# compix/Monte-Carlo-Raytracer

Measured on AMD Instinct MI355X. Metric: Mpaths/sec + achieved HBM GB/s, San-Miguel 1920x1080 at 1/2/4/8 MI355X, higher is better.
Workload: dtype f32; 1 GPU; san_miguel_proxy 1920x1080, unidirectional PT, maxDepth 2, random sampler, 1 spp per step, box-filter accumulate; width=1920, height=1080, triangles=9984786, max_depth=2, global_batch=1, bvh=RadeonRays-identical SAH, device build, parallelism=tile-split 8-row bands x 1 + 1 RCCL band gather, frames_per_launch=32, max_frames_per_call=32

## Files before the change

### monte-carlo-raytracer_amd/csrc/mcrt_kernels.hip

```cpp
#include <algorithm>

#include <rocprim/device/device_scan.hpp>

#include "mcrt_device.h"
#include "mcrt_internal.h"
#include "mcrt_traverse.h"
#include "mcrt_shading.h"

#ifndef SHADE0_BLOCK
#define SHADE0_BLOCK 512
#endif
#define SHADEN_BLOCK 256
#define MCRT_EXT_GROUPS 24

template <bool ANY, int LAY>
__global__ __launch_bounds__(64) void k_trace_rays(TraceCtx c, const mcrt_ray* __restrict__ rays, int n,
                                                   const int* __restrict__ countDev,
                                                   mcrt_intersection* __restrict__ hits, int* __restrict__ occl) {
    __shared__ __attribute__((aligned(16))) uint32_t lds[STACK_LDS * 64];
    if (countDev) n = min(n, *countDev);
    const int lane = threadIdx.x;
    const int i = blockIdx.x * 64 + lane;
    if (i >= n) return;
    const mcrt_ray rr = rays[i];
// ... 288 lines not shown

__global__ __launch_bounds__(64) void k_walk_resume(TraceCtx c, const float4* __restrict__ qO,
                                                    const float4* __restrict__ qD, float4* __restrict__ hitOut) {
    __shared__ __attribute__((aligned(16))) uint32_t lds[STACK_LDS * 64];
    const int n = *c.suspendCount;
    if ((int)blockIdx.x * 64 >= n) return;
    const int lane = threadIdx.x;
    const int j = blockIdx.x * 64 + lane;
    if (j >= n) return;
    const float4* sv = c.suspend + (size_t)j * MCRT_SUSPEND_F4;
    const float4 s0 = sv[0], s1 = sv[1];
    const int i = __float_as_int(s0.x);
    uint32_t* stk = lds + lane;
    uint32_t col = 0;
    for (int k = 0; k < STACK_LDS / 4; ++k) {
        const float4 e = sv[2 + k];
        if (k == 0) col = __float_as_uint(e.x);
        stk[(4 * k) * 64] = k == 0 ? QREF_DONE : __float_as_uint(e.x);
        stk[(4 * k + 1) * 64] = __float_as_uint(e.y);
        stk[(4 * k + 2) * 64] = __float_as_uint(e.z);
        stk[(4 * k + 3) * 64] = __float_as_uint(e.w);
    }
    QWalk w{__float_as_uint(s0.y), s0.z, s0.w, s1.x, __float_as_int(s1.y), __float_as_int(s1.z), __float_as_int(s1.w)};
    const float4 o = qO[i], d = qD[i];
    TraceRay r;
    r.o = ld3(o);
    r.d = ld3(d);
    r.tmax = RT_MAX_TRACE_F;
    r.mask = -1;
    uint32_t* spill = raySpill(c, (int)(col >> 6), (int)(col & 63));
    qwalk<false, -2>(c, r, safeInvDir(r.d), stk, spill, w);
    hitOut[i] = qwalkClosest(c, r, stk, spill, w);
}

template <int LAY0, int LAY1>
__global__ __launch_bounds__(64) void k_extend_pair(TraceCtx cc, TraceCtx c, const int* __restrict__ count0,
                                                    const float4* __restrict__ qO0, const float4* __restrict__ qD0,
                                                    float4* __restrict__ hit0, const int* __restrict__ count1,
                                                    const float4* __restrict__ qO1, const float4* __restrict__ qD1,
                                                    float4* __restrict__ hit1, const uint32_t* __restrict__ perm1) {
    __shared__ __attribute__((aligned(16))) uint32_t lds[STACK_LDS * 64];
    const int n0 = *count0;
    const int b0 = (n0 + 63) >> 6;
    const int lane = threadIdx.x;
    TraceRay r;
    r.tmax = RT_MAX_TRACE_F;
    r.mask = -1;
    float t;
    if ((int)blockIdx.x < b0) {
        const int blk = xcdRemap(blockIdx.x, b0);
        const int i = blk * 64 + lane;
        if (LAY0 == LAY_PLAIN && cc.packet) {
            const bool valid = i < n0;
            r.o = valid ? ld3(qO0[i]) : splat3(0.0f);
            r.d = valid ? ld3(qD0[i]) : f3{0.0f, 0.0f, 1.0f};
            const int tri = traversePacket<false>(cc.nodes, r, valid, t);
            if (valid) hit0[i] = closestRecord(cc.nodes, r, tri, t);
            return;
        }
        if (i >= n0) return;
        r.o = ld3(qO0[i]);
        r.d = ld3(qD0[i]);
        hit0[i] = traceClosest<LAY0>(cc, r, lds + lane, raySpill(cc, blk, lane), t);
    } else {
        const int n1 = *count1;
        const int b1 = (n1 + 63) >> 6;
        if ((int)blockIdx.x - b0 >= b1) return;
        const int j = xcdRemap((int)blockIdx.x - b0, b1) * 64 + lane;
        if (perm1 == nullptr) {
            if (j >= n1) return;
            r.o = ld3(qO1[j]);
            r.d = ld3(qD1[j]);
            closestOrSuspend<LAY1>(c, r, lds + lane, (int)blockIdx.x * 64 + lane, j, hit1);
            return;
        }
        if (j >= n1) return;
        const int i = (int)perm1[j];
        r.o = ld3(qO1[i]);
        r.d = ld3(qD1[i]);
        closestOrSuspend<LAY1>(c, r, lds + lane, (int)blockIdx.x * 64 + lane, i, hit1);
    }
}

struct ShadeOut {
    bool pushS, pushE;
    float4 sO, sD, sL;
    float4 eO, eD, eT;
};

template <bool LOD = false, bool EXT = true, bool RR = false>
MCRT_DEV f3 shadePath(const SceneArgs& s, const FrameArgs& f, int bounce, int pix, float4 hit, f3 dir, f3 throughput,
                      int prevFlags, ShadeOut& o, f3 ro = f3{0, 0, 0}, f3 dxDir = f3{0, 0, 0}, f3 dyDir = f3{0, 0, 0}) {
    f3 add = splat3(0.0f);
    const int shapeIdx = __float_as_int(hit.z), primIdx = __float_as_int(hit.w);
    if (shapeIdx < 0 || s.numLights <= 0) return add;
    const mcrt_shape shape = tableEntry(s.shapes, shapeIdx);
    f3 dpdu, dpdv;
    Frame si = computeSurfaceInteraction(s, shape, shapeIdx, primIdx, f2{hit.x, hit.y}, LOD ? &dpdu : nullptr,
                                         LOD ? &dpdv : nullptr);
    TexLod lod{{0.0f, 0.0f}, {0.0f, 0.0f}, false};
    if (LOD) lod = surfaceUVDifferentials(si, dpdu, dpdv, ro, dxDir, dyDir);
    const f3 wo = -dir;
    const bool isBackfacing = cl_dot(si.gn, wo) < 0.0f;
    const float traceErrorOffset = isBackfacing ? -RT_TRACE_OFFSET_F : RT_TRACE_OFFSET_F;
    const int materialId = shape.materialId;
    mcrt_material mat;
    if (materialId != -1) {
        mat = tableEntry(s.materials, materialId);
        if (mat.uber_normalMapId != -1) applyNormalMapping(s, mat.uber_normalMapId, si, lod);
    }
    if (bounce == 0) throughput = splat3(1.0f);
    if (shape.lightID != -1 && (bounce == 0 || (prevFlags & BSDF_SPECULAR) == BSDF_SPECULAR)) {
        const mcrt_light& L = s.lights[shape.lightID];
        f3 Le = splat3(0.0f);
        if ((L.type == MCRT_DISK_AREA_LIGHT || L.type == MCRT_TRIANGLE_MESH_AREA_LIGHT) && cl_dot(si.gn, wo) > 0.0f)
            Le = ld3(L.intensity);
        return throughput * Le;
    }
    int px = pix, frame = f.frame;
    if (f.batch > 1) {
        const int k = (int)((uint32_t)pix / (f.W * f.H));
        px = pix - k * (int)(f.W * f.H);
        frame += k;
    }
    Sampler sampler = makeSampler(f.sampler, (uint32_t)px, frame, bounce, f.W, f.H, s.sobol);
    const bool isUber = materialId != -1 && mat.type == 0;
    Uber um;
    if (isUber) um = uberProps(s, mat, si.uv, lod);
    {
        uint32_t lightIdx = (uint32_t)floorf(getSample1D(sampler) * s.numLights);
        lightIdx %= (uint32_t)s.numLights;
        const f2 u = getSample2D(sampler);
        const mcrt_light light = s.lights[lightIdx];
        const LightSample ls = sampleLightLi(s, light, si, traceErrorOffset, u);
        float lightPdf = ls.pdf * light.choicePdf;
        f3 L = splat3(0.0f);
        if (materialId != -1) {
            f3 bsdf = isUber ? evaluateUberBSDF(um, si, wo, ls.wi) : splat3(0.0f);
            bsdf *= absDot(ls.wi, si.sn);
            if (!isNearZero(lightPdf)) L = cl_div(ls.Li * bsdf, lightPdf);
        }
        const f3 term = throughput * L;
        if (term.x != 0.0f || term.y != 0.0f || term.z != 0.0f) {
            if (ls.shadowSet) {
                o.pushS = true;
                o.sO = make_float4(ls.shadowO.x, ls.shadowO.y, ls.shadowO.z, ls.shadowT);
                o.sD = make_float4(ls.wi.x, ls.wi.y, ls.wi.z, __int_as_float(pix));
                o.sL = make_float4(term.x, term.y, term.z, 0.0f);
            } else {
                add = term * 0.0f;
            }
        }
    }
    if (EXT && bounce + 1 < f.maxDepth) {
        const f2 bsdfSample = getSample2D(sampler);
        if (isUber) {
            f3 wi;
            float pdf;
            int sampledType;
            f3 bsdfBounce = sampleUberBSDF(um, si, bsdfSample, wo, &wi, &pdf, &sampledType);
            if (!(isNearZero(pdf) || isBlack(bsdfBounce))) {
                bsdfBounce = cl_div(bsdfBounce, pdf);
                const f3 tp = bsdfBounce * absDot(wi, si.sn);
                const f3 nt = throughput * tp;
                float off = traceErrorOffset;
                if ((sampledType & BSDF_TRANSMISSION) != 0 && cl_dot(si.gn, wi) * cl_sign(off) < 0.0f) off *= -1.0f;
                const f3 no = si.p + si.gn * off;
                bool alive = true;
                f3 tp1 = nt;
                if (RR && bounce + 1 >= f.rrStartDepth) {
                    const float qr = fmaxf(0.05f, 1.0f - fmaxf(nt.x, fmaxf(nt.y, nt.z)));
                    const float ur = (float)wangHash((uint32_t)px * 9781u + (uint32_t)frame * 6271u + (uint32_t)bounce) * 0x1p-32f;
                    alive = ur >= qr;
                    tp1 = cl_div(nt, (1.0f - qr));
                }
                if (alive) {
                    o.pushE = true;
                    o.eO = make_float4(no.x, no.y, no.z, __int_as_float(pix));
                    o.eD = make_float4(wi.x, wi.y, wi.z, __int_as_float(sampledType));
                    o.eT = make_float4(tp1.x, tp1.y, tp1.z, 0.0f);
                }
            }
        }
    }
    return add;
}

template <bool LOD, bool RR>
__global__ __launch_bounds__(SHADE0_BLOCK) void k_shade0(SceneArgs s, FrameArgs f, const mcrt_camera* __restrict__ camp,
                                                const float4* __restrict__ hits, float4* __restrict__ radiance,
                                                QueueArgs q) {
    const int lane = threadIdx.x & 63;
    const int tileAll = orderedTileAll(f, xcdRemap(blockIdx.x, gridDim.x) * (SHADE0_BLOCK / 64) + (int)(threadIdx.x >> 6));
    int k, tile, pi = lane;
    if (f.shadePack && f.batch > 1) {
        packedPath(f, tileAll, lane, k, tile, pi);
    } else {
        splitTileFrame(f, tileAll, k, tile);
    }
    int x = 0, y = 0;
    bool valid = k < f.batch && tile < f.numTiles && tilePixel(f, tile, pi, x, y);
    __shared__ int ldsWave[SHADE0_BLOCK / 64 + 1];
    __shared__ int ldsGroup[MCRT_EXT_GROUPS + 1];
    ShadeOut o;
    o.pushS = o.pushE = false;
    o.eD = make_float4(0.0f, 0.0f, 0.0f, 0.0f);
    if (valid) {
        const mcrt_camera& cam = camp[k];
        const int pix = k * (int)(f.W * f.H) + y * (int)f.W + x;
        const f3 dir = cameraDir(cam, x, y);
        f3 dx = splat3(0.0f), dy = splat3(0.0f);
        if (LOD) cameraDiffDirs(cam, x, y, dx, dy);
        const f3 add = shadePath<LOD, true, RR>(s, f, 0, pix, hits[hitSlot(f, tile, pi, k, x, y)], dir, splat3(1.0f), 0,
                                                o, ld3(cam.pos), dx, dy);
        radiance[pix] = make_float4(add.x, add.y, add.z, 0.0f);
    }
    const int ss = blockAppend<SHADE0_BLOCK / 64>(q.shadowCount, o.pushS, ldsWave);
    if (o.pushS) { q.sO[ss] = o.sO; q.sD[ss] = o.sD; q.sL[ss] = o.sL; }
    int oct = (o.eD.x < 0.0f ? 1 : 0) | (o.eD.y < 0.0f ? 2 : 0) | (o.eD.z < 0.0f ? 4 : 0);
    {
        const float ax = fabsf(o.eD.x), ay = fabsf(o.eD.y), az = fabsf(o.eD.z);
        oct = oct * 3 + (ax >= ay && ax >= az ? 0 : ay >= az ? 1 : 2);
    }
    const int es = blockAppendGroupedLds<MCRT_EXT_GROUPS>(q.extCountOut, o.pushE, oct, ldsGroup);
    if (o.pushE) { q.eOout[es] = o.eO; q.eDout[es] = o.eD; q.eTout[es] = o.eT; }
}

template <bool LAST, bool RR>
__global__ __launch_bounds__(SHADEN_BLOCK) void k_shadeN(SceneArgs s, FrameArgs f, int bounce, const int* __restrict__ countIn,
                                                const float4* __restrict__ qO, const float4* __restrict__ qD,
                                                const float4* __restrict__ qT, const float4* __restrict__ hits,
                                                float4* __restrict__ radiance, QueueArgs q) {
    const int n = *countIn;
    __shared__ int ldsWave[SHADEN_BLOCK / 64 + 1];
    __shared__ int ldsGroup[(SHADEN_BLOCK / 64) * 8 + 1];
    if ((int)blockIdx.x * SHADEN_BLOCK >= n) return;
    const int i = xcdRemap(blockIdx.x, (n + SHADEN_BLOCK - 1) / SHADEN_BLOCK) * SHADEN_BLOCK + threadIdx.x;
    ShadeOut o;
    o.pushS = o.pushE = false;
    o.eD = make_float4(0.0f, 0.0f, 0.0f, 0.0f);
    if (i < n) {
        const float4 O = qO[i], D = qD[i], Tp = qT[i];
        const int pix = __float_as_int(O.w);
        const f3 add = shadePath<false, !LAST, RR>(s, f, bounce, pix, hits[i], ld3(D), ld3(Tp), __float_as_int(D.w), o);
        if (add.x != 0.0f || add.y != 0.0f || add.z != 0.0f || add.x != add.x) {
            float4 r = radiance[pix];
            r.x += add.x; r.y += add.y; r.z += add.z;
            radiance[pix] = r;
        }
    }
    const int ss = blockAppend<SHADEN_BLOCK / 64>(q.shadowCount, o.pushS, ldsWave);
    if (o.pushS) { q.sO[ss] = o.sO; q.sD[ss] = o.sD; q.sL[ss] = o.sL; }
    if (LAST) return;
    const int oct = (o.eD.x < 0.0f ? 1 : 0) | (o.eD.y < 0.0f ? 2 : 0) | (o.eD.z < 0.0f ? 4 : 0);
    const int es = blockAppendGrouped<SHADEN_BLOCK / 64, 8>(q.extCountOut, o.pushE, oct, ldsGroup);
    if (o.pushE) { q.eOout[es] = o.eO; q.eDout[es] = o.eD; q.eTout[es] = o.eT; }
}

__global__ __launch_bounds__(256) void k_aov(SceneArgs s, FrameArgs f, const mcrt_camera* __restrict__ camp,
                                             const float4* __restrict__ hits, int which, float4* __restrict__ out) {
    const int lane = threadIdx.x & 63;
    const int tile = (blockIdx.x * blockDim.x + threadIdx.x) >> 6;
    int x, y;
    if (tile >= f.numTiles || !tilePixel(f, tile, lane, x, y)) return;
    const int pix = y * (int)f.W + x;
    const int stride = which == MCRT_AOV_TEXTURE_LOD ? 3 : 1;
    float4* o = out + (size_t)pix * stride;
    for (int k = 0; k < stride; ++k) o[k] = make_float4(0.0f, 0.0f, 0.0f, 0.0f);
    const float4 hit = hits[hitSlot(f, tile, lane, 0, x, y)];
    const int shapeIdx = __float_as_int(hit.z), primIdx = __float_as_int(hit.w);
    if (shapeIdx < 0) return;
    const mcrt_camera& cam = *camp;
    f3 dpdu, dpdv, dx, dy;
    const Frame si = computeSurfaceInteraction(s, shapeIdx, primIdx, f2{hit.x, hit.y}, &dpdu, &dpdv);
    cameraDiffDirs(cam, x, y, dx, dy);
    TexLod L = surfaceUVDifferentials(si, dpdu, dpdv, ld3(cam.pos), dx, dy);
    const int materialId = s.shapes[shapeIdx].materialId;
    if (which == MCRT_AOV_TEXTURE_LOD) {
        float lod = 0.0f;
        f4 c = f4{0.0f, 0.0f, 0.0f, 0.0f};
        if (materialId != -1 && s.materials[materialId].uber_diffuseTexId != -1) {
            const int t = s.materials[materialId].uber_diffuseTexId;
            const mcrt_texture_desc tex = s.textures[t];
            lod = mipLod(tex, L.duvdx, L.duvdy);
            c = readTexLodDesc(s, tex, si.uv, lod);
        }
        o[0] = make_float4(L.duvdx.x, L.duvdx.y, L.duvdy.x, L.duvdy.y);
        o[1] = make_float4(lod, __int_as_float(shapeIdx), si.uv.x, si.uv.y);
        o[2] = make_float4(c.x, c.y, c.z, c.w);
    } else {
        L.on = f.textureLod != 0;
        if (materialId != -1 && s.materials[materialId].type == 0) {
            const Uber u = uberProps(s, s.materials[materialId], si.uv, L);
            o[0] = make_float4(u.Kd.x, u.Kd.y, u.Kd.z, u.opacity.x);
        }
    }
}

template <bool MOTION>
__device__ __forceinline__ void guidesPixel(const SceneArgs& s, const FrameArgs& f, const mcrt_camera* __restrict__ camp,
                                            const float4* __restrict__ hits, float4* __restrict__ normalPlane,
                                            float4* __restrict__ albedoDepth, const PrevPose* __restrict__ prev,
                                            float4* __restrict__ motion, float4* __restrict__ prevNormal) {
    const int lane = threadIdx.x & 63;
    const int tile = (blockIdx.x * blockDim.x + threadIdx.x) >> 6;
    int x, y;
    if (tile >= f.numTiles || !tilePixel(f, tile, lane, x, y)) return;
    const int pix = y * (int)f.W + x;
    const float4 hit = hits[hitSlot(f, tile, lane, 0, x, y)];
    const int shapeIdx = __float_as_int(hit.z), primIdx = __float_as_int(hit.w);
    if (shapeIdx < 0) {
        normalPlane[pix] = make_float4(0.0f, 0.0f, 0.0f, 0.0f);
        albedoDepth[pix] = make_float4(0.0f, 0.0f, 0.0f, -1.0f);
        if (MOTION) {
            motion[pix] = make_float4(0.0f, 0.0f, 0.0f, 0.0f);
            prevNormal[pix] = make_float4(0.0f, 0.0f, 0.0f, 0.0f);
        }
        return;
    }
    const mcrt_camera& cam = *camp;
    f3 dpdu, dpdv, dx, dy;
    const Frame si = computeSurfaceInteraction(s, shapeIdx, primIdx, f2{hit.x, hit.y}, &dpdu, &dpdv);
    cameraDiffDirs(cam, x, y, dx, dy);
    TexLod L = surfaceUVDifferentials(si, dpdu, dpdv, ld3(cam.pos), dx, dy);
    L.on = f.textureLod != 0;
    f3 kd = f3{0.0f, 0.0f, 0.0f};
    const int materialId = s.shapes[shapeIdx].materialId;
    if (materialId != -1 && s.materials[materialId].type == 0) kd = uberProps(s, s.materials[materialId], si.uv, L).Kd;
    const f3 v = si.p - ld3(cam.pos);
    f3 n = si.sn;
    float off = cl_dot(n, v);
    const bool flipped = off > 0.0f;
    if (flipped) {
        n = f3{-n.x, -n.y, -n.z};
        off = -off;
    }
    normalPlane[pix] = make_float4(n.x, n.y, n.z, off);
    albedoDepth[pix] = make_float4(kd.x, kd.y, kd.z, cl_length(v));
    if (MOTION) {
// ... 691 lines not shown
```

### monte-carlo-raytracer_amd/csrc/mcrt_shading.h

```cpp
#pragma once
#include "mcrt_device.h"
#include "mcrt_internal.h"

MCRT_DEV bool tilePixel(const FrameArgs& f, int tile, int lane, int& x, int& y) {
    const int tb = tile / f.tilesX, tx = tile - tb * f.tilesX;
    const int bpb = f.bandRows >> 3;
    const int gb = (tb / bpb) * bpb * f.numBands + f.bandIndex * bpb + (tb % bpb);
    x = tx * 8 + (lane & 7);
    y = gb * 8 + (lane >> 3);
    return x < (int)f.W && y < (int)f.H;
}

MCRT_DEV int orderedTileAll(const FrameArgs& f, int tileAll) {
    if (!f.tileOrder) return tileAll;
    const int slot = tileAll / f.batch, part = tileAll - slot * f.batch;
    return slot < f.numTiles ? (int)f.tileOrder[slot] * f.batch + part : tileAll;
}

MCRT_DEV void splitTileFrame(const FrameArgs& f, int tileAll, int& k, int& tile) {
    if (f.tileMajor) {
        tile = tileAll / f.batch;
        k = tileAll - tile * f.batch;
    } else {
        k = tileAll / f.numTiles;
// ... 76 lines not shown

MCRT_DEV f4 readTexLodDesc(const SceneArgs& s, const mcrt_texture_desc& tex, f2 uv, float lod) {
    if (lod < 1e-8f || tex.numMipLevels < 2) return readTexDesc(s, tex, uv);
    if (lod >= (float)(tex.numMipLevels - 1)) {
        mcrt_texture_desc top = tex;
        uint16_t w = tex.width, h = tex.height;
        int off = 0;
        for (int i = 0; i < tex.numMipLevels - 1; ++i) {
            off += w * h * 4;
            w = (uint16_t)max(w / 2, 1);
            h = (uint16_t)max(h / 2, 1);
        }
        top.width = 1;
        top.height = 1;
        top.memOffset += off;
        return readTexDesc(s, top, uv);
    }
    const int lower = (int)floorf(lod);
    uint16_t w = tex.width, h = tex.height;
    int off = 0;
    for (int i = 0; i < lower; ++i) {
        off += w * h * 4;
        w = (uint16_t)max(w / 2, 1);
        h = (uint16_t)max(h / 2, 1);
    }
    mcrt_texture_desc lo = tex, hi = tex;
    lo.width = w;
    lo.height = h;
    lo.memOffset += off;
    const int offHi = off + w * h * 4;
    hi.width = (uint16_t)max(w / 2, 1);
    hi.height = (uint16_t)max(h / 2, 1);
    hi.memOffset += offHi;
    const f4 v0 = readTexDesc(s, lo, uv), v1 = readTexDesc(s, hi, uv);
    const float t = lod - (float)lower;
    return f4{fmaf(v1.x - v0.x, t, v0.x), fmaf(v1.y - v0.y, t, v0.y), fmaf(v1.z - v0.z, t, v0.z),
              fmaf(v1.w - v0.w, t, v0.w)};
}

MCRT_DEV f4 readTexL(const SceneArgs& s, int texId, f2 uv, const TexLod& L) {
    if (!L.on) return readTex(s, texId, uv);
    const mcrt_texture_desc tex = tableEntry(s.textures, texId);
    return readTexLodDesc(s, tex, uv, mipLod(tex, L.duvdx, L.duvdy));
}

MCRT_DEV bool solve2x2(float a00, float a01, float a10, float a11, f2 B, f2* x) {
    const float det = a00 * a11 - a10 * a01;
    if (fabsf(det) < 1e-8f) return false;
    *x = f2{cl_div(a11 * B.x - a01 * B.y, det), cl_div(a00 * B.y - a10 * B.x, det)};
    return true;
}

MCRT_DEV void cameraDiffDirs(const mcrt_camera& cam, int x, int y, f3& dx, f3& dy) {
    const f2 r = f2{cl_div(1.0f, (float)cam.width), cl_div(1.0f, (float)cam.height)};
    const f2 uv = f2{(float)x * r.x, (float)y * r.y};
    dx = lerpDirection(ld3(cam.r00), ld3(cam.r10), ld3(cam.r11), ld3(cam.r01), uv.x + r.x, uv.y);
    dy = lerpDirection(ld3(cam.r00), ld3(cam.r10), ld3(cam.r11), ld3(cam.r01), uv.x, uv.y + r.y);
}

MCRT_DEV Uber uberProps(const SceneArgs& s, const mcrt_material& material, f2 uv, const TexLod& L = TexLod{{0, 0}, {0, 0}, false},
                        bool* nonDelta = nullptr) {
    Uber u;
    const f4 Kd_opacity = material.uber_diffuseTexId != -1 ? readTexL(s, material.uber_diffuseTexId, uv, L) : f4{1.0f, 1.0f, 1.0f, 1.0f};
    u.Kd = Kd_opacity.xyz * ld3(material.uber_kd);
    const f3 glossy = material.uber_glossyTexId != -1 ? readTexL(s, material.uber_glossyTexId, uv, L).xyz : splat3(1.0f);
    u.Ks = glossy * ld3(material.uber_ks);
    u.Kr = (material.uber_specReflectionTexId != -1 ? readTexL(s, material.uber_specReflectionTexId, uv, L).xyz : splat3(1.0f)) *
           ld3(material.uber_kr);
    u.Kt.xyz = (material.uber_transmissionTexId != -1 ? readTexL(s, material.uber_transmissionTexId, uv, L).xyz : splat3(1.0f)) *
               ld3(material.uber_kt);
    u.Kt.w = material.uber_kt.w;
    const f3 opTex = material.uber_opacityTexId != -1 ? readTexL(s, material.uber_opacityTexId, uv, L).xyz : splat3(1.0f);
    u.opacity = opTex * ld3(material.uber_opacity) * Kd_opacity.w;
    if (nonDelta) {
        const f3 Kd = material.uber_diffuseTexId != -1 ? Kd_opacity.xyz : ld3(material.uber_kd);
        const f3 Ks = material.uber_glossyTexId != -1 ? glossy : ld3(material.uber_ks);
        const f3 op = material.uber_opacityTexId != -1 ? opTex : ld3(material.uber_opacity);
        const f3 kd = Kd * op, ks = Ks * op;
        *nonDelta = !isBlack(kd) || !isBlack(ks);
    }
    u.roughness = material.uber_roughnessTexId != -1 ? readTexL(s, material.uber_roughnessTexId, uv, L).xy
                                                      : f2{material.uber_roughness.x, material.uber_roughness.y};
    u.eta = material.uber_iorTexId != -1 ? readTexL(s, material.uber_iorTexId, uv, L).x : material.uber_eta;
    u.roughness = f2{roughnessToAlpha(u.roughness.x), roughnessToAlpha(u.roughness.y)};
    return u;
}

template <int NW>
MCRT_DEV int blockAppend(int* counter, bool pred, int* ldsWave ) {
    const unsigned long long m = __ballot(pred);
    const int lane = threadIdx.x & 63, wv = threadIdx.x >> 6;
    if (lane == 0) ldsWave[wv] = __popcll(m);
    __syncthreads();
    if (threadIdx.x == 0) {
        int sum = 0;
        for (int w = 0; w < NW; ++w) {
            const int c = ldsWave[w];
            ldsWave[w] = sum;
            sum += c;
        }
        ldsWave[NW] = sum ? atomicAdd(counter, sum) : 0;
    }
    __syncthreads();
    const unsigned lo = (unsigned)m, hi = (unsigned)(m >> 32);
    const int prefix = __builtin_amdgcn_mbcnt_hi(hi, __builtin_amdgcn_mbcnt_lo(lo, 0u));
    const int slot = ldsWave[NW] + ldsWave[wv] + prefix;
    __syncthreads();
    return slot;
}

template <int NW, int G>
MCRT_DEV int blockAppendGrouped(int* counter, bool pred, int group, int* lds) {
    const int lane = threadIdx.x & 63, wv = threadIdx.x >> 6;
    unsigned long long mine = 0;
#pragma unroll
    for (int g = 0; g < G; ++g) {
        const unsigned long long m = __ballot(pred && group == g);
        if (g == group) mine = m;
        if (lane == 0) lds[g * NW + wv] = __popcll(m);
    }
    __syncthreads();
    if (threadIdx.x == 0) {
        int sum = 0;
        for (int i = 0; i < G * NW; ++i) {
            const int c = lds[i];
            lds[i] = sum;
            sum += c;
        }
        lds[G * NW] = sum ? atomicAdd(counter, sum) : 0;
    }
    __syncthreads();
    const int prefix = __builtin_amdgcn_mbcnt_hi((unsigned)(mine >> 32), __builtin_amdgcn_mbcnt_lo((unsigned)mine, 0u));
    const int slot = lds[G * NW] + (pred ? lds[group * NW + wv] : 0) + prefix;
    __syncthreads();
    return slot;
}

template <int G>
MCRT_DEV int blockAppendGroupedLds(int* counter, bool pred, int group, int* lds) {
    for (int g = threadIdx.x; g < G; g += blockDim.x) lds[g] = 0;
    __syncthreads();
    const int local = pred ? atomicAdd(&lds[group], 1) : 0;
    __syncthreads();
    if (threadIdx.x == 0) {
        int sum = 0;
        for (int g = 0; g < G; ++g) {
            const int c = lds[g];
            lds[g] = sum;
            sum += c;
        }
        lds[G] = sum ? atomicAdd(counter, sum) : 0;
    }
    __syncthreads();
    const int slot = lds[G] + (pred ? lds[group] : 0) + local;
    __syncthreads();
    return slot;
}

MCRT_DEV int waveAppend(int* counter, bool pred) {
    const unsigned long long m = __ballot(pred);
    if (m == 0) return 0;
    const int lane = threadIdx.x & 63;
    const int leader = __ffsll((long long)m) - 1;
    int base = 0;
    if (lane == leader) base = atomicAdd(counter, __popcll(m));
    base = __shfl(base, leader);
// ... 187 lines not shown
```

### monte-carlo-raytracer_amd/mcrt/lib.py

```python
import ctypes
import weakref
import os

import numpy as np

from . import PKG_DIR
from . import types as T

_DEFAULT_LIB = os.path.join(os.path.dirname(PKG_DIR), "libmcrt.so")
LIB_PATH = os.environ.get("MCRT_LIB_PATH") or _DEFAULT_LIB
HEADER = os.path.join(os.path.dirname(os.path.dirname(PKG_DIR)), "include", "mcrt_capi.h")

_c = ctypes
_vp = _c.c_void_p
_lib = None

SIGNATURES = {
    "mcrt_version": (_c.c_char_p, []),
    "mcrt_last_error": (_c.c_char_p, [_vp]),
    "mcrt_ctx_create": (_c.c_int, [_c.c_int, _c.POINTER(_vp)]),
    "mcrt_ctx_destroy": (_c.c_int, [_vp]),
    "mcrt_ctx_synchronize": (_c.c_int, [_vp]),
    "mcrt_ctx_set_stream": (_c.c_int, [_vp, _vp]),
    "mcrt_ctx_set_profiling": (_c.c_int, [_vp, _c.c_int]),
# ... 276 lines not shown
        return rec

    def builder(self):
        b = _c.c_int32()
        _check(lib().mcrt_accel_builder(self.h, _c.byref(b)), self.ctx.h)
        return b.value

    def info(self):
        nn, nb, ms, nt = _c.c_uint64(), _c.c_uint64(), _c.c_double(), _c.c_uint32()
        _check(lib().mcrt_accel_info(self.h, _c.byref(nn), _c.byref(nb), _c.byref(ms), _c.byref(nt)), self.ctx.h)
        return {"nodes": nn.value, "bytes": nb.value, "build_ms": ms.value, "triangles": nt.value}

    def update_lights(self, lights):
        self._lights = np.ascontiguousarray(lights)
        _check(lib().mcrt_scene_update_lights(self.h, _p(self._lights), len(self._lights)), self.ctx.h)

    def update_materials(self, mats):
        self._mats = np.ascontiguousarray(mats)
        _check(lib().mcrt_scene_update_materials(self.h, _p(self._mats), len(self._mats)), self.ctx.h)

    def update_shapes(self, shapes):
        self._shapes = np.ascontiguousarray(shapes)
        _check(lib().mcrt_scene_update_shapes(self.h, _p(self._shapes), len(self._shapes)), self.ctx.h)

    def update_transforms(self, shapes, world_to_local=None):
        self._shapes = np.ascontiguousarray(shapes)
        w2l = None if world_to_local is None else np.ascontiguousarray(world_to_local, np.float32)
        _check(lib().mcrt_accel_update_transforms(self.h, _p(self._shapes), len(self._shapes), _p(w2l)), self.ctx.h)

    def motion_snapshot(self):
        _check(lib().mcrt_scene_motion_snapshot(self.h), self.ctx.h)

    def update_info(self):
        path, ms = _c.c_int32(), _c.c_double()
        _check(lib().mcrt_accel_update_info(self.h, _c.byref(path), _c.byref(ms)), self.ctx.h)
        return {"path": path.value, "ms": ms.value}

    def trace_closest(self, rays_dev_ptr, n, hits_dev_ptr):
        _check(lib().mcrt_trace_closest(self.h, rays_dev_ptr, n, hits_dev_ptr), self.ctx.h)

    def trace_any(self, rays_dev_ptr, n, out_dev_ptr):
        _check(lib().mcrt_trace_any(self.h, rays_dev_ptr, n, out_dev_ptr), self.ctx.h)

    def trace_count(self, any_hit, rays_dev_ptr, count_dev_ptr, maxrays, out_dev_ptr, wait_event=None,
                    want_event=False):
        ev = _vp()
        f = lib().mcrt_trace_any_count if any_hit else lib().mcrt_trace_closest_count
        _check(f(self.h, rays_dev_ptr, count_dev_ptr, maxrays, out_dev_ptr, wait_event,
                 _c.byref(ev) if want_event else None), self.ctx.h)
        return ev.value if want_event else None

    def close(self):
        if self.h:
            lib().mcrt_scene_destroy(self.h)
            self.h = None

    def __del__(self):
        try:
            self.close()
        except Exception:
            pass


class FrameBuffer:
    def __init__(self, ctx, width, height):
        self.ctx = ctx
        self.W, self.H = width, height
        h = _vp()
        _check(lib().mcrt_framebuffer_create(ctx.h, width, height, _c.byref(h)), ctx.h)
        self.h = h
        ctx._adopt(self)

    def set_frames_in_flight(self, n):
        _check(lib().mcrt_framebuffer_set_frames_in_flight(self.h, n), self.ctx.h)

    def render(self, dscene, cam, frame=0, max_depth=2, sampler=T.SAMPLER_RANDOM, rr=False, rr_start=3,
               band_rows=8, num_bands=1, band_index=0, integrator=T.INTEGRATOR_PT, texture_lod=False):
        p = T.FrameParams(frame, max_depth, sampler, 1 if rr else 0, rr_start, band_rows, num_bands, band_index,
                          integrator, 1 if texture_lod else 0)
        cam = np.ascontiguousarray(cam)
        _check(lib().mcrt_render_frame(dscene.h, self.h, _p(cam), _c.byref(p)), self.ctx.h)

    def render_frames(self, dscene, cams, frame=0, max_depth=2, sampler=T.SAMPLER_RANDOM, rr=False, rr_start=3,
                      band_rows=8, num_bands=1, band_index=0, integrator=T.INTEGRATOR_PT):
        p = T.FrameParams(frame, max_depth, sampler, 1 if rr else 0, rr_start, band_rows, num_bands, band_index,
                          integrator, 0)
        cams = _records(cams)
        _check(lib().mcrt_render_frames(dscene.h, self.h, _p(cams), len(cams), _c.byref(p)), self.ctx.h)

    def accumulate_frames(self, filters, frame):
        filters = _records(filters)
        _check(lib().mcrt_accumulate_frames(self.h, _p(filters), len(filters), frame), self.ctx.h)

    def render_aov(self, dscene, cam, aov=T.AOV_ALBEDO, texture_lod=False):
        p = T.FrameParams(0, 1, T.SAMPLER_RANDOM, 0, 3, 8, 1, 0, T.INTEGRATOR_PT, 1 if texture_lod else 0)
        cam = np.ascontiguousarray(cam)
        shape = (self.H, self.W, 3, 4) if aov == T.AOV_TEXTURE_LOD else (self.H, self.W, 4)
        out = np.zeros(shape, np.float32)
        _check(lib().mcrt_render_aov(dscene.h, self.h, _p(cam), _c.byref(p), aov, _p(out)), self.ctx.h)
        return out

    def accumulate(self, filt, frame):
        filt = np.ascontiguousarray(filt)
        _check(lib().mcrt_accumulate(self.h, _p(filt), frame), self.ctx.h)

    def postprocess(self, denoise=False, radius=1, sigma_spatial=1.0, sigma_range=0.1, tonemap=False,
                    min_luminance=2.0):
        p = T.PostprocessParams(1 if denoise else 0, radius, sigma_spatial, sigma_range, 1 if tonemap else 0,
                                min_luminance)
        _check(lib().mcrt_postprocess(self.h, _c.byref(p)), self.ctx.h)

    def render_guides(self, dscene, cam, texture_lod=False, band_rows=8, num_bands=1, band_index=0):
        p = T.FrameParams(0, 1, T.SAMPLER_RANDOM, 0, 3, band_rows, num_bands, band_index, T.INTEGRATOR_PT,
                          1 if texture_lod else 0)
        cam = np.ascontiguousarray(cam)
        _check(lib().mcrt_render_guides(dscene.h, self.h, _p(cam), _c.byref(p)), self.ctx.h)

    def render_guides_motion(self, dscene, cam, texture_lod=False, band_rows=8, num_bands=1, band_index=0):
        p = T.FrameParams(0, 1, T.SAMPLER_RANDOM, 0, 3, band_rows, num_bands, band_index, T.INTEGRATOR_PT,
                          1 if texture_lod else 0)
        cam = np.ascontiguousarray(cam)
        _check(lib().mcrt_render_guides_motion(dscene.h, self.h, _p(cam), _c.byref(p)), self.ctx.h)

    def set_motion(self, motion_ptr, prev_normal_ptr):
        _check(lib().mcrt_framebuffer_set_motion(self.h, motion_ptr, prev_normal_ptr), self.ctx.h)

    def read_motion(self, which):
        out = np.zeros((self.H, self.W, 4), np.float32)
        _check(lib().mcrt_framebuffer_read_motion(self.h, which, _p(out), out.nbytes, None), self.ctx.h)
        return out

    def set_guides(self, normal_plane_ptr, albedo_depth_ptr):
        _check(lib().mcrt_framebuffer_set_guides(self.h, normal_plane_ptr, albedo_depth_ptr), self.ctx.h)

    def enable_moments(self, on=True):
        _check(lib().mcrt_framebuffer_set_moments_enabled(self.h, 1 if on else 0), self.ctx.h)

    def set_moments(self, m1m2_ptr, frames):
        _check(lib().mcrt_framebuffer_set_moments(self.h, m1m2_ptr, int(frames)), self.ctx.h)

    GUIDE_SHAPES = {T.GUIDE_NORMAL_PLANE: (4,), T.GUIDE_ALBEDO_DEPTH: (4,), T.GUIDE_MOMENTS: (2,),
                    T.GUIDE_FILTERED_VARIANCE: ()}

    def read_guides(self, which):
        out = np.zeros((self.H, self.W) + self.GUIDE_SHAPES[which], np.float32)
        _check(lib().mcrt_framebuffer_read_guides(self.h, which, _p(out), out.nbytes, None), self.ctx.h)
        return out

    def denoise_guided(self, levels=5, sigma_normal=0.1, sigma_depth=0.02, sigma_luminance=4.0, use_variance=True,
                       demodulate_albedo=True, tonemap=False, min_luminance=2.0):
        p = T.GuidedDenoiseParams(levels, sigma_normal, sigma_depth, sigma_luminance, 1 if use_variance else 0,
                                  1 if demodulate_albedo else 0, 1 if tonemap else 0, min_luminance)
        _check(lib().mcrt_denoise_guided(self.h, _c.byref(p)), self.ctx.h)

    def temporal_accumulate(self, cam, alpha=0.2, alpha_moments=0.2, max_history=32, min_history=4,
                            normal_threshold=0.1, plane_threshold=0.01, demodulate_albedo=True):
        p = T.TemporalParams(alpha, alpha_moments, max_history, min_history, normal_threshold, plane_threshold,
                             1 if demodulate_albedo else 0)
        cam = np.ascontiguousarray(cam)
        _check(lib().mcrt_temporal_accumulate(self.h, _p(cam), _c.byref(p)), self.ctx.h)

    def temporal_accumulate_motion(self, cam, alpha=0.2, alpha_moments=0.2, max_history=32, min_history=4,
                                   normal_threshold=0.1, plane_threshold=0.01, demodulate_albedo=True):
        p = T.TemporalParams(alpha, alpha_moments, max_history, min_history, normal_threshold, plane_threshold,
                             1 if demodulate_albedo else 0)
        cam = np.ascontiguousarray(cam)
        _check(lib().mcrt_temporal_accumulate_motion(self.h, _p(cam), _c.byref(p)), self.ctx.h)

    def temporal_reset(self):
# ... 205 lines not shown
```

Before: 1932 Mpaths/s.

## Split shading into direct and extension phases with piecewise material loads

Splits the monolithic shadePath into shadeDirect and shadeExtend, so the shadow-ray queue append happens before the BSDF sampling for the extension ray. Material records are now read in 16-byte pieces on demand instead of copying the full 128-byte struct, and throughput is loaded lazily from the queue. Empty asm 'pin' barriers are added to control scheduling and register live ranges. The goal is lower register pressure and less memory traffic in the shade kernels. In exchange, the ShadeState struct must carry the surface frame and Uber properties across the block-wide append, which may raise live registers at that point. It also adds a texture_lod option to the Python render_frames call.

```diff
diff --git a/monte-carlo-raytracer_amd/csrc/mcrt_kernels.hip b/monte-carlo-raytracer_amd/csrc/mcrt_kernels.hip
--- a/monte-carlo-raytracer_amd/csrc/mcrt_kernels.hip
+++ b/monte-carlo-raytracer_amd/csrc/mcrt_kernels.hip
@@ -394,15 +394,32 @@
     }
 }
 
-struct ShadeOut {
-    bool pushS, pushE;
-    float4 sO, sD, sL;
-    float4 eO, eD, eT;
+struct ShadowRay {
+    bool push;
+    float4 o, d, l;
 };
-
-template <bool LOD = false, bool EXT = true, bool RR = false>
-MCRT_DEV f3 shadePath(const SceneArgs& s, const FrameArgs& f, int bounce, int pix, float4 hit, f3 dir, f3 throughput,
-                      int prevFlags, ShadeOut& o, f3 ro = f3{0, 0, 0}, f3 dxDir = f3{0, 0, 0}, f3 dyDir = f3{0, 0, 0}) {
+struct ExtRay {
+    bool push;
+    float4 o, d, t;
+};
+struct ShadeState {
+    bool ext;
+    Frame si;
+    Uber um;
+    f3 wo;
+    float traceErrorOffset;
+    f2 bsdfSample;
+    int px, frame;
+};
+
+MCRT_DEV f3 pathThroughput(int bounce, const float4* throughputAt) {
+    return bounce == 0 ? splat3(1.0f) : ld3(*throughputAt);
+}
+
+template <bool LOD = false, bool EXT = true, bool LIGHT_IN_PLACE = true>
+MCRT_DEV f3 shadeDirect(const SceneArgs& s, const FrameArgs& f, int bounce, int pix, float4 hit, f3 dir,
+                        const float4* throughputAt, int prevFlags, ShadowRay& sr, ShadeState& st, f3 ro = f3{0, 0, 0},
+                        f3 dxDir = f3{0, 0, 0}, f3 dyDir = f3{0, 0, 0}) {
     f3 add = splat3(0.0f);
     const int shapeIdx = __float_as_int(hit.z), primIdx = __float_as_int(hit.w);
     if (shapeIdx < 0 || s.numLights <= 0) return add;
@@ -410,24 +427,30 @@
     f3 dpdu, dpdv;
     Frame si = computeSurfaceInteraction(s, shape, shapeIdx, primIdx, f2{hit.x, hit.y}, LOD ? &dpdu : nullptr,
                                          LOD ? &dpdv : nullptr);
+    pin(si.p); pin(si.gn); pin(si.sn); pin(si.sdpdu); pin(si.sdpdv); pin(si.uv);
     TexLod lod{{0.0f, 0.0f}, {0.0f, 0.0f}, false};
-    if (LOD) lod = surfaceUVDifferentials(si, dpdu, dpdv, ro, dxDir, dyDir);
-    const f3 wo = -dir;
+    if (LOD) {
+        lod = surfaceUVDifferentials(si, dpdu, dpdv, ro, dxDir, dyDir);
+        pin(lod.duvdx); pin(lod.duvdy);
+    }
+    f3 wo = -dir;
+    pin(wo);
     const bool isBackfacing = cl_dot(si.gn, wo) < 0.0f;
     const float traceErrorOffset = isBackfacing ? -RT_TRACE_OFFSET_F : RT_TRACE_OFFSET_F;
     const int materialId = shape.materialId;
-    mcrt_material mat;
+    const MatAt mat{s.materials, materialId};
+    int matTypeId = -1;
     if (materialId != -1) {
-        mat = tableEntry(s.materials, materialId);
-        if (mat.uber_normalMapId != -1) applyNormalMapping(s, mat.uber_normalMapId, si, lod);
-    }
-    if (bounce == 0) throughput = splat3(1.0f);
+        matTypeId = matType(mat);
+        const int normalMapId = matNormalMapId(mat);
+        if (normalMapId != -1) applyNormalMapping(s, normalMapId, si, lod);
+    }
     if (shape.lightID != -1 && (bounce == 0 || (prevFlags & BSDF_SPECULAR) == BSDF_SPECULAR)) {
         const mcrt_light& L = s.lights[shape.lightID];
         f3 Le = splat3(0.0f);
         if ((L.type == MCRT_DISK_AREA_LIGHT || L.type == MCRT_TRIANGLE_MESH_AREA_LIGHT) && cl_dot(si.gn, wo) > 0.0f)
             Le = ld3(L.intensity);
-        return throughput * Le;
+        return pathThroughput(bounce, throughputAt) * Le;
     }
     int px = pix, frame = f.frame;
     if (f.batch > 1) {
@@ -436,67 +459,87 @@
         frame += k;
     }
     Sampler sampler = makeSampler(f.sampler, (uint32_t)px, frame, bounce, f.W, f.H, s.sobol);
-    const bool isUber = materialId != -1 && mat.type == 0;
+    uint32_t lightIdx = (uint32_t)floorf(getSample1D(sampler) * s.numLights);
+    lightIdx %= (uint32_t)s.numLights;
+    const f2 u = getSample2D(sampler);
+    f2 bsdfSample{0.0f, 0.0f};
+    if (EXT && bounce + 1 < f.maxDepth) {
+        bsdfSample = getSample2D(sampler);
+        pin(bsdfSample);
+    }
+    mcrt_light lightRecord;
+    if (!LIGHT_IN_PLACE) lightRecord = s.lights[lightIdx];
+    const mcrt_light& light = LIGHT_IN_PLACE ? s.lights[lightIdx] : lightRecord;
+    LightSample ls = sampleLightLi(s, light, si, traceErrorOffset, u);
+    float lightPdf = ls.pdf * light.choicePdf;
+    pin(ls.Li); pin(ls.wi); pin(ls.shadowO); pin(ls.shadowT); pin(lightPdf);
+    const bool isUber = materialId != -1 && matTypeId == 0;
     Uber um;
     if (isUber) um = uberProps(s, mat, si.uv, lod);
     {
-        uint32_t lightIdx = (uint32_t)floorf(getSample1D(sampler) * s.numLights);
-        lightIdx %= (uint32_t)s.numLights;
-        const f2 u = getSample2D(sampler);
-        const mcrt_light light = s.lights[lightIdx];
-        const LightSample ls = sampleLightLi(s, light, si, traceErrorOffset, u);
-        float lightPdf = ls.pdf * light.choicePdf;
         f3 L = splat3(0.0f);
         if (materialId != -1) {
             f3 bsdf = isUber ? evaluateUberBSDF(um, si, wo, ls.wi) : splat3(0.0f);
             bsdf *= absDot(ls.wi, si.sn);
             if (!isNearZero(lightPdf)) L = cl_div(ls.Li * bsdf, lightPdf);
         }
-        const f3 term = throughput * L;
+        const f3 term = pathThroughput(bounce, throughputAt) * L;
         if (term.x != 0.0f || term.y != 0.0f || term.z != 0.0f) {
             if (ls.shadowSet) {
-                o.pushS = true;
-                o.sO = make_float4(ls.shadowO.x, ls.shadowO.y, ls.shadowO.z, ls.shadowT);
-                o.sD = make_float4(ls.wi.x, ls.wi.y, ls.wi.z, __int_as_float(pix));
-                o.sL = make_float4(term.x, term.y, term.z, 0.0f);
+                sr.push = true;
+                sr.o = make_float4(ls.shadowO.x, ls.shadowO.y, ls.shadowO.z, ls.shadowT);
+                sr.d = make_float4(ls.wi.x, ls.wi.y, ls.wi.z, __int_as_float(pix));
+                sr.l = make_float4(term.x, term.y, term.z, 0.0f);
             } else {
                 add = term * 0.0f;
             }
         }
     }
-    if (EXT && bounce + 1 < f.maxDepth) {
-        const f2 bsdfSample = getSample2D(sampler);
-        if (isUber) {
-            f3 wi;
-            float pdf;
-            int sampledType;
-            f3 bsdfBounce = sampleUberBSDF(um, si, bsdfSample, wo, &wi, &pdf, &sampledType);
-            if (!(isNearZero(pdf) || isBlack(bsdfBounce))) {
-                bsdfBounce = cl_div(bsdfBounce, pdf);
-                const f3 tp = bsdfBounce * absDot(wi, si.sn);
-                const f3 nt = throughput * tp;
-                float off = traceErrorOffset;
-                if ((sampledType & BSDF_TRANSMISSION) != 0 && cl_dot(si.gn, wi) * cl_sign(off) < 0.0f) off *= -1.0f;
-                const f3 no = si.p + si.gn * off;
-                bool alive = true;
-                f3 tp1 = nt;
-                if (RR && bounce + 1 >= f.rrStartDepth) {
-                    const float qr = fmaxf(0.05f, 1.0f - fmaxf(nt.x, fmaxf(nt.y, nt.z)));
-                    const float ur = (float)wangHash((uint32_t)px * 9781u + (uint32_t)frame * 6271u + (uint32_t)bounce) * 0x1p-32f;
-                    alive = ur >= qr;
-                    tp1 = cl_div(nt, (1.0f - qr));
-                }
-                if (alive) {
-                    o.pushE = true;
-                    o.eO = make_float4(no.x, no.y, no.z, __int_as_float(pix));
-                    o.eD = make_float4(wi.x, wi.y, wi.z, __int_as_float(sampledType));
-                    o.eT = make_float4(tp1.x, tp1.y, tp1.z, 0.0f);
-                }
-            }
-        }
+    if (EXT && bounce + 1 < f.maxDepth && isUber) {
+        st.ext = true;
+        st.si = si;
+        st.um = um;
+        st.wo = wo;
+        st.traceErrorOffset = traceErrorOffset;
+        st.bsdfSample = bsdfSample;
+        st.px = px;
+        st.frame = frame;
     }
     return add;
 }
+
+template <bool RR = false>
+MCRT_DEV void shadeExtend(const FrameArgs& f, int bounce, int pix, const float4* throughputAt, ShadeState& st,
+                          ExtRay& er) {
+    const Frame& si = st.si;
+    f3 wi;
+    float pdf;
+    int sampledType;
+    f3 bsdfBounce = sampleUberBSDF(st.um, si, st.bsdfSample, st.wo, &wi, &pdf, &sampledType);
+    if (!(isNearZero(pdf) || isBlack(bsdfBounce))) {
+        bsdfBounce = cl_div(bsdfBounce, pdf);
+        const f3 tp = bsdfBounce * absDot(wi, si.sn);
+        const f3 nt = pathThroughput(bounce, throughputAt) * tp;
+        float off = st.traceErrorOffset;
+        if ((sampledType & BSDF_TRANSMISSION) != 0 && cl_dot(si.gn, wi) * cl_sign(off) < 0.0f) off *= -1.0f;
+        const f3 no = si.p + si.gn * off;
+        bool alive = true;
+        f3 tp1 = nt;
+        if (RR && bounce + 1 >= f.rrStartDepth) {
+            const float qr = fmaxf(0.05f, 1.0f - fmaxf(nt.x, fmaxf(nt.y, nt.z)));
+            const float ur = (float)wangHash((uint32_t)st.px * 9781u + (uint32_t)st.frame * 6271u + (uint32_t)bounce) * 0x1p-32f;
+            alive = ur >= qr;
+            tp1 = cl_div(nt, (1.0f - qr));
+        }
+        if (alive) {
+            er.push = true;
+            er.o = make_float4(no.x, no.y, no.z, __int_as_float(pix));
+            er.d = make_float4(wi.x, wi.y, wi.z, __int_as_float(sampledType));
+            er.t = make_float4(tp1.x, tp1.y, tp1.z, 0.0f);
+        }
+    }
+}
+
 
 template <bool LOD, bool RR>
 __global__ __launch_bounds__(SHADE0_BLOCK) void k_shade0(SceneArgs s, FrameArgs f, const mcrt_camera* __restrict__ camp,
@@ -514,28 +557,33 @@
     bool valid = k < f.batch && tile < f.numTiles && tilePixel(f, tile, pi, x, y);
     __shared__ int ldsWave[SHADE0_BLOCK / 64 + 1];
     __shared__ int ldsGroup[MCRT_EXT_GROUPS + 1];
-    ShadeOut o;
-    o.pushS = o.pushE = false;
-    o.eD = make_float4(0.0f, 0.0f, 0.0f, 0.0f);
+    ShadowRay sr;
+    ShadeState st;
+    sr.push = st.ext = false;
+    int pix = 0;
     if (valid) {
         const mcrt_camera& cam = camp[k];
-        const int pix = k * (int)(f.W * f.H) + y * (int)f.W + x;
+        pix = k * (int)(f.W * f.H) + y * (int)f.W + x;
         const f3 dir = cameraDir(cam, x, y);
         f3 dx = splat3(0.0f), dy = splat3(0.0f);
         if (LOD) cameraDiffDirs(cam, x, y, dx, dy);
-        const f3 add = shadePath<LOD, true, RR>(s, f, 0, pix, hits[hitSlot(f, tile, pi, k, x, y)], dir, splat3(1.0f), 0,
-                                                o, ld3(cam.pos), dx, dy);
+        const f3 add = shadeDirect<LOD, true>(s, f, 0, pix, hits[hitSlot(f, tile, pi, k, x, y)], dir, nullptr, 0, sr, st,
+                                              ld3(cam.pos), dx, dy);
         radiance[pix] = make_float4(add.x, add.y, add.z, 0.0f);
     }
-    const int ss = blockAppend<SHADE0_BLOCK / 64>(q.shadowCount, o.pushS, ldsWave);
-    if (o.pushS) { q.sO[ss] = o.sO; q.sD[ss] = o.sD; q.sL[ss] = o.sL; }
-    int oct = (o.eD.x < 0.0f ? 1 : 0) | (o.eD.y < 0.0f ? 2 : 0) | (o.eD.z < 0.0f ? 4 : 0);
+    const int ss = blockAppend<SHADE0_BLOCK / 64>(q.shadowCount, sr.push, ldsWave);
+    if (sr.push) { q.sO[ss] = sr.o; q.sD[ss] = sr.d; q.sL[ss] = sr.l; }
+    ExtRay er;
+    er.push = false;
+    er.d = make_float4(0.0f, 0.0f, 0.0f, 0.0f);
+    if (st.ext) shadeExtend<RR>(f, 0, pix, nullptr, st, er);
+    int oct = (er.d.x < 0.0f ? 1 : 0) | (er.d.y < 0.0f ? 2 : 0) | (er.d.z < 0.0f ? 4 : 0);
     {
-        const float ax = fabsf(o.eD.x), ay = fabsf(o.eD.y), az = fabsf(o.eD.z);
+        const float ax = fabsf(er.d.x), ay = fabsf(er.d.y), az = fabsf(er.d.z);
         oct = oct * 3 + (ax >= ay && ax >= az ? 0 : ay >= az ? 1 : 2);
     }
-    const int es = blockAppendGroupedLds<MCRT_EXT_GROUPS>(q.extCountOut, o.pushE, oct, ldsGroup);
-    if (o.pushE) { q.eOout[es] = o.eO; q.eDout[es] = o.eD; q.eTout[es] = o.eT; }
+    const int es = blockAppendGroupedLds<MCRT_EXT_GROUPS>(q.extCountOut, er.push, oct, ldsGroup);
+    if (er.push) { q.eOout[es] = er.o; q.eDout[es] = er.d; q.eTout[es] = er.t; }
 }
 
 template <bool LAST, bool RR>
@@ -548,25 +596,30 @@
     __shared__ int ldsGroup[(SHADEN_BLOCK / 64) * 8 + 1];
     if ((int)blockIdx.x * SHADEN_BLOCK >= n) return;
     const int i = xcdRemap(blockIdx.x, (n + SHADEN_BLOCK - 1) / SHADEN_BLOCK) * SHADEN_BLOCK + threadIdx.x;
-    ShadeOut o;
-    o.pushS = o.pushE = false;
-    o.eD = make_float4(0.0f, 0.0f, 0.0f, 0.0f);
+    ShadowRay sr;
+    ShadeState st;
+    sr.push = st.ext = false;
+    int pix = 0;
     if (i < n) {
-        const float4 O = qO[i], D = qD[i], Tp = qT[i];
-        const int pix = __float_as_int(O.w);
-        const f3 add = shadePath<false, !LAST, RR>(s, f, bounce, pix, hits[i], ld3(D), ld3(Tp), __float_as_int(D.w), o);
+        const float4 O = qO[i], D = qD[i];
+        pix = __float_as_int(O.w);
+        const f3 add = shadeDirect<false, !LAST, false>(s, f, bounce, pix, hits[i], ld3(D), qT + i, __float_as_int(D.w), sr, st);
         if (add.x != 0.0f || add.y != 0.0f || add.z != 0.0f || add.x != add.x) {
             float4 r = radiance[pix];
             r.x += add.x; r.y += add.y; r.z += add.z;
             radiance[pix] = r;
         }
     }
-    const int ss = blockAppend<SHADEN_BLOCK / 64>(q.shadowCount, o.pushS, ldsWave);
-    if (o.pushS) { q.sO[ss] = o.sO; q.sD[ss] = o.sD; q.sL[ss] = o.sL; }
+    const int ss = blockAppend<SHADEN_BLOCK / 64>(q.shadowCount, sr.push, ldsWave);
+    if (sr.push) { q.sO[ss] = sr.o; q.sD[ss] = sr.d; q.sL[ss] = sr.l; }
     if (LAST) return;
-    const int oct = (o.eD.x < 0.0f ? 1 : 0) | (o.eD.y < 0.0f ? 2 : 0) | (o.eD.z < 0.0f ? 4 : 0);
-    const int es = blockAppendGrouped<SHADEN_BLOCK / 64, 8>(q.extCountOut, o.pushE, oct, ldsGroup);
-    if (o.pushE) { q.eOout[es] = o.eO; q.eDout[es] = o.eD; q.eTout[es] = o.eT; }
+    ExtRay er;
+    er.push = false;
+    er.d = make_float4(0.0f, 0.0f, 0.0f, 0.0f);
+    if (st.ext) shadeExtend<RR>(f, bounce, pix, qT + i, st, er);
+    const int oct = (er.d.x < 0.0f ? 1 : 0) | (er.d.y < 0.0f ? 2 : 0) | (er.d.z < 0.0f ? 4 : 0);
+    const int es = blockAppendGrouped<SHADEN_BLOCK / 64, 8>(q.extCountOut, er.push, oct, ldsGroup);
+    if (er.push) { q.eOout[es] = er.o; q.eDout[es] = er.d; q.eTout[es] = er.t; }
 }
 
 __global__ __launch_bounds__(256) void k_aov(SceneArgs s, FrameArgs f, const mcrt_camera* __restrict__ camp,
diff --git a/monte-carlo-raytracer_amd/csrc/mcrt_shading.h b/monte-carlo-raytracer_amd/csrc/mcrt_shading.h
--- a/monte-carlo-raytracer_amd/csrc/mcrt_shading.h
+++ b/monte-carlo-raytracer_amd/csrc/mcrt_shading.h
@@ -182,6 +182,65 @@
     u.roughness = material.uber_roughnessTexId != -1 ? readTexL(s, material.uber_roughnessTexId, uv, L).xy
                                                       : f2{material.uber_roughness.x, material.uber_roughness.y};
     u.eta = material.uber_iorTexId != -1 ? readTexL(s, material.uber_iorTexId, uv, L).x : material.uber_eta;
+    u.roughness = f2{roughnessToAlpha(u.roughness.x), roughnessToAlpha(u.roughness.y)};
+    return u;
+}
+
+MCRT_DEV void pin(float& x) { asm volatile("" : "+v"(x)); }
+MCRT_DEV void pin(f2& v) {
+    float x = v.x, y = v.y;
+    pin(x); pin(y);
+    v = f2{x, y};
+}
+MCRT_DEV void pin(f3& v) {
+    float x = v.x, y = v.y, z = v.z;
+    pin(x); pin(y); pin(z);
+    v = f3{x, y, z};
+}
+MCRT_DEV void pin(f4& v) {
+    float x = v.x, y = v.y, z = v.z, w = v.w;
+    pin(x); pin(y); pin(z); pin(w);
+    v = f4{x, y, z, w};
+}
+
+struct MatAt {
+    const mcrt_material* tab;
+    int id;
+};
+enum { MAT_KD, MAT_KS, MAT_KR, MAT_KT, MAT_OPACITY, MAT_ROUGHNESS_ETA_TYPE, MAT_TEX_NDGS, MAT_TEX_TORI };
+static_assert(sizeof(mcrt_material) == 8 * sizeof(float4), "mcrt_material is eight 16-byte pieces");
+MCRT_DEV float4 matPiece(const MatAt& m, int piece) {
+    return tableEntry(reinterpret_cast<const float4*>(m.tab), m.id * 8 + piece);
+}
+MCRT_DEV int matType(const MatAt& m) { return __float_as_int(matPiece(m, MAT_ROUGHNESS_ETA_TYPE).w); }
+MCRT_DEV int matNormalMapId(const MatAt& m) { return __float_as_int(matPiece(m, MAT_TEX_NDGS).x); }
+
+MCRT_DEV Uber uberProps(const SceneArgs& s, const MatAt& material, f2 uv, const TexLod& L = TexLod{{0, 0}, {0, 0}, false}) {
+    Uber u;
+    const float4 ndgs = matPiece(material, MAT_TEX_NDGS), tori = matPiece(material, MAT_TEX_TORI);
+    const int diffuseTexId = __float_as_int(ndgs.y), glossyTexId = __float_as_int(ndgs.z);
+    const int specReflectionTexId = __float_as_int(ndgs.w), transmissionTexId = __float_as_int(tori.x);
+    const int opacityTexId = __float_as_int(tori.y), roughnessTexId = __float_as_int(tori.z);
+    const int iorTexId = __float_as_int(tori.w);
+    const f4 Kd_opacity = diffuseTexId != -1 ? readTexL(s, diffuseTexId, uv, L) : f4{1.0f, 1.0f, 1.0f, 1.0f};
+    u.Kd = Kd_opacity.xyz * ld3(matPiece(material, MAT_KD));
+    pin(u.Kd);
+    const f3 glossy = glossyTexId != -1 ? readTexL(s, glossyTexId, uv, L).xyz : splat3(1.0f);
+    u.Ks = glossy * ld3(matPiece(material, MAT_KS));
+    pin(u.Ks);
+    u.Kr = (specReflectionTexId != -1 ? readTexL(s, specReflectionTexId, uv, L).xyz : splat3(1.0f)) *
+           ld3(matPiece(material, MAT_KR));
+    pin(u.Kr);
+    const float4 kt = matPiece(material, MAT_KT);
+    u.Kt.xyz = (transmissionTexId != -1 ? readTexL(s, transmissionTexId, uv, L).xyz : splat3(1.0f)) * ld3(kt);
+    u.Kt.w = kt.w;
+    pin(u.Kt);
+    const f3 opTex = opacityTexId != -1 ? readTexL(s, opacityTexId, uv, L).xyz : splat3(1.0f);
+    u.opacity = opTex * ld3(matPiece(material, MAT_OPACITY)) * Kd_opacity.w;
+    pin(u.opacity);
+    const float4 ret = matPiece(material, MAT_ROUGHNESS_ETA_TYPE);
+    u.roughness = roughnessTexId != -1 ? readTexL(s, roughnessTexId, uv, L).xy : f2{ret.x, ret.y};
+    u.eta = iorTexId != -1 ? readTexL(s, iorTexId, uv, L).x : ret.z;
     u.roughness = f2{roughnessToAlpha(u.roughness.x), roughnessToAlpha(u.roughness.y)};
     return u;
 }
diff --git a/monte-carlo-raytracer_amd/mcrt/lib.py b/monte-carlo-raytracer_amd/mcrt/lib.py
--- a/monte-carlo-raytracer_amd/mcrt/lib.py
+++ b/monte-carlo-raytracer_amd/mcrt/lib.py
@@ -382,9 +382,9 @@
         _check(lib().mcrt_render_frame(dscene.h, self.h, _p(cam), _c.byref(p)), self.ctx.h)
 
     def render_frames(self, dscene, cams, frame=0, max_depth=2, sampler=T.SAMPLER_RANDOM, rr=False, rr_start=3,
-                      band_rows=8, num_bands=1, band_index=0, integrator=T.INTEGRATOR_PT):
+                      band_rows=8, num_bands=1, band_index=0, integrator=T.INTEGRATOR_PT, texture_lod=False):
         p = T.FrameParams(frame, max_depth, sampler, 1 if rr else 0, rr_start, band_rows, num_bands, band_index,
-                          integrator, 0)
+                          integrator, 1 if texture_lod else 0)
         cams = _records(cams)
         _check(lib().mcrt_render_frames(dscene.h, self.h, _p(cams), len(cams), _c.byref(p)), self.ctx.h)
 
```

Measured after the change: 1945 Mpaths/s (median of 6 runs). Within noise of the previous version (+0.7%).
